# Gancheekim/ATM-VFI

Measured on AMD Instinct MI355X. Metric: interpolated frames/s at 1080p (network_base, bs=1), higher is better.
Workload: dtype f32 (contractions as fp16 hi/lo split x3 MFMA, fp32 accumulate; ~22 significand bits)

## Files before the change

### atm-vfi_amd/csrc/conv3x3_planes.hip

```cpp
#include "conv3_common.h"

#include <stdlib.h>

#ifdef ATMVFI_STAMP
static unsigned long long* g_planes_stamp = nullptr;
extern "C" void atmvfi_debug_set_planes_stamp_buffer(void* p) { g_planes_stamp = (unsigned long long*)p; }
#ifdef ATMVFI_STAMP_KSTEP
#define PDBG(bit) ((a.dbg & (bit)) != 0)
#else
#define PDBG(bit) false
#endif
#define PSTAMP_DECL unsigned long long st_[8] = {0, 0, 0, 0, 0, 0, 0, 0}; unsigned long long st_epi = 0; unsigned long long st_t0 = __builtin_amdgcn_s_memtime();
#define TSTAMP(k) { __builtin_amdgcn_sched_barrier(0); const unsigned long long t1_ = __builtin_amdgcn_s_memtime(); st_[k] += t1_ - st_t0; st_t0 = t1_; __builtin_amdgcn_sched_barrier(0); }
#ifdef ATMVFI_STAMP_KSTEP
#define PSTAMP(k) TSTAMP(k)
#else
#define PSTAMP(k)
#endif
#else
#define PDBG(bit) false
#define PSTAMP_DECL
#define PSTAMP(k)
#define TSTAMP(k)
#endif

namespace {

struct Conv3PDev {
    const _Float16* in_hi;
    const _Float16* in_lo;
    long long in_rows;
    int N, H, W, Cin;
    const _Float16* w_hi;
    const _Float16* w_lo;
    int wrows, cf, tail;
    int Cout;
    float* out;
    int out_ld;
    const float* bias;
    const float* prelu;
    _Float16* out_hi;
    _Float16* out_lo;
    long long plane_rows;
    int out_c0;
    const float* plane_prelu;
    _Float16* out_hi2;
    _Float16* out_lo2;
    long long plane_rows2;
    int out_c02;
    int out_cmin;
    int tiles_x, tiles_y, nblocks, tchunk;
    int vblocks;
    unsigned dm_nblocks, ds_nblocks, dm_perimg, ds_perimg, dm_grp, ds_grp, dm_rows, ds_rows;
    int ksplit, cps;
    long long part_stride;
    const _Float16* h2_w;
    float* h2_out;
    long long h2_plane;
    unsigned long long* stamp;
    int dbg;
};

constexpr int HALO_PIX = HW_ * HW_;
constexpr int HALO_PLANE_PIECES = (HALO_PIX + 15) / 16;
constexpr int HALO_LO = HALO_PLANE_PIECES * 1024;
constexpr int HALO_BYTES = 2 * HALO_LO;

constexpr int planes_const_floats(int BN) { return (3 * BN + 63) / 64 * 64; }
constexpr int ring_slots(int wn) {
    const int free_bytes = 160 * 1024 - 2 * HALO_BYTES - 2 * planes_const_floats(16 * wn) * 4;
    const int n = free_bytes / (2 * 16 * wn * 64);
    return n > 5 ? 5 : n;
}
template <int N>
__device__ __forceinline__ void wait_vm() { asm volatile("s_waitcnt vmcnt(%0)" ::"n"(N) : "memory"); }
__device__ __forceinline__ void dma16(const unsigned char* src, unsigned char* lds_wave_base) {
    __builtin_amdgcn_global_load_lds((const __attribute__((address_space(1))) void*)src,
                                     (__attribute__((address_space(3))) void*)lds_wave_base, 16, 0, 0);
}

template <int BN>
__device__ __forceinline__ void dma_planes_consts(const float* bias, const float* slope, const float* plane_slope, int Cout, int n0, float* cst,
                                                  int wave, int lane) {
    constexpr int NPIECE = (3 * BN + 63) / 64;
    static_assert(NPIECE <= 8, "one piece per wave");
    const int piece = wave % NPIECE;
    const int t = piece * 64 + lane;
    const int row = t / BN;
    const int col = n0 + t - row * BN;
    const float* src = row == 0 ? bias : row == 1 ? slope : plane_slope;
    const float* p = (src && row < 3 && col < Cout) ? src + col : &kEpilogueDefaults[row == 0 ? 0 : 1];
    __builtin_amdgcn_global_load_lds((const __attribute__((address_space(1))) void*)p,
                                     (__attribute__((address_space(3))) void*)(cst + piece * 64), 4, 0, 0);
}

template <int WN>
__global__ __launch_bounds__(512, 1) void conv3x3_planes_kernel(const Conv3PDev a) {
    fp16_saturate_on();
    constexpr int BN = 16 * WN;
    constexpr int WSLOT = 2 * BN * 64;
    constexpr int SW = (2 * WN + 7) / 8;
    constexpr int NB = ring_slots(WN);
    constexpr int LA = NB - 1;
    constexpr int CSTF = planes_const_floats(BN);
    extern __shared__ __attribute__((aligned(16))) unsigned char smem[];
    const unsigned halo0 = lds_offset(smem);
    const unsigned ring0 = halo0 + 2 * HALO_BYTES;
    float* cst_base = reinterpret_cast<float*>(smem + 2 * HALO_BYTES + NB * WSLOT);

    const int tid = threadIdx.x;
    const int lane = tid & 63;
    const int wave = __builtin_amdgcn_readfirstlane(tid >> 6);
    const int grp = wave >> 2;
    const int r = lane & 15;
    const int g = lane >> 4;

    const _Float16* in_hi = a.in_hi;
    const _Float16* in_lo = a.in_lo;
    const _Float16* w_hi = a.w_hi;
    const _Float16* w_lo = a.w_lo;
    float* out_f32 = a.out;
    int nfull = a.cf >> 5;
    int ktail = a.tail;
    if (a.ksplit > 1) {
        const int sp = blockIdx.y;
        const int rem = nfull - a.cps * a.ksplit;
        const int c0 = sp * a.cps + (sp < rem ? sp : rem);
        const bool last = sp == a.ksplit - 1;
        in_hi += (long long)c0 * a.in_rows * 32;
        in_lo += (long long)c0 * a.in_rows * 32;
        w_hi += (long long)c0 * 9 * a.wrows * 32;
        w_lo += (long long)c0 * 9 * a.wrows * 32;
        nfull = a.cps + (sp < rem ? 1 : 0);
        ktail = last ? ktail : 0;
        out_f32 += sp * a.part_stride;
    }

    const int grid = gridDim.x;
    const int per_img = a.tiles_x * a.tiles_y;
    auto fdiv = [](int n, unsigned m, unsigned sh) -> int { return (int)((__umulhi((unsigned)n, m) + (unsigned)n) >> sh); };
    auto decode = [&](int v, int& t_img, int& t_ox0, int& t_oy0, int& t_n0) -> bool {
        int sgrp, nblk, L;
        if (a.ksplit > 1) {
            sgrp = fdiv(v, a.dm_nblocks, a.ds_nblocks);
            nblk = v - sgrp * a.nblocks;
            L = sgrp;
        } else {
            const int slot = v >> 3;
// ... 158 lines not shown
#pragma unroll
            for (int i = 0; i < 2; ++i) {
                const int p = prow + i * HW_ + ((dtail >> (TAIL ? 8 * T : 0)) & 0xff);
                const unsigned addr = halo0 + (unsigned)hcur + (unsigned)(p * 64 + (swz64(p) << 4));
                lds_read16<0>(xh[i], addr);
                lds_read16<HALO_LO>(xl[i], addr);
            }
        }
        const unsigned wa = wfrag + (unsigned)rd_off;
        if (!PDBG(16)) static_for<0, WN>([&](auto jc) {
            constexpr int j = decltype(jc)::value;
            lds_read16<j * 1024>(wh[j], wa);
            lds_read16<j * 1024 + BN * 64>(wl[j], wa);
        });
        rd_off = rd_off + WSLOT == NB * WSLOT ? 0 : rd_off + WSLOT;
        PSTAMP(1)
        if (!PDBG(2)) issue_weights();
        if constexpr (!TAIL && T < 6) {
            if (!PDBG(1)) issue_halo(std::integral_constant<int, T>{});
        }
        if constexpr (TAIL && T < 2) {
            if (!PDBG(1)) {
                issue_halo(std::integral_constant<int, 3 * T>{});
                issue_halo(std::integral_constant<int, 3 * T + 1>{});
                issue_halo(std::integral_constant<int, 3 * T + 2>{});
            }
        }
        PSTAMP(2)
        if constexpr (FIRST && T < LA - 1) {
        } else {
            constexpr int lo = T + 1 - LA > 0 ? T + 1 - LA : 0;
            constexpr int hi = T < 5 ? T : 5;
            constexpr int halos = !TAIL ? (hi >= lo ? hi - lo + 1 : 0) : (lo <= 0 ? 3 : 0) + ((lo <= 1 && T >= 1) ? 3 : 0);
            if (!PDBG(4)) wait_vm<(!TAIL && T == 8) ? (LA - 1) * SW : (LA - 1) * SW + halos>();
        }
        PSTAMP(3)
        asm volatile("s_waitcnt lgkmcnt(0)"
                     : "+v"(xh[0]), "+v"(xh[1]), "+v"(xl[0]), "+v"(xl[1]));
#pragma unroll
        for (int j = 0; j < WN; ++j) asm volatile("" : "+v"(wh[j]), "+v"(wl[j]));
        __builtin_amdgcn_sched_barrier(0);
        PSTAMP(4)
        __builtin_amdgcn_s_barrier();
        __builtin_amdgcn_sched_barrier(0);
        PSTAMP(5)
        if (!PDBG(8)) __builtin_amdgcn_s_setprio(1);
        static_for<0, WN>([&](auto jc) {
            constexpr int j = decltype(jc)::value;
            cor[0][j] = __builtin_amdgcn_mfma_f32_16x16x32_f16(wl[j], xh[0], cor[0][j], 0, 0, 0);
            cor[1][j] = __builtin_amdgcn_mfma_f32_16x16x32_f16(wl[j], xh[1], cor[1][j], 0, 0, 0);
            acc[0][j] = __builtin_amdgcn_mfma_f32_16x16x32_f16(wh[j], xh[0], acc[0][j], 0, 0, 0);
            acc[1][j] = __builtin_amdgcn_mfma_f32_16x16x32_f16(wh[j], xh[1], acc[1][j], 0, 0, 0);
            cor[0][j] = __builtin_amdgcn_mfma_f32_16x16x32_f16(wh[j], xl[0], cor[0][j], 0, 0, 0);
            cor[1][j] = __builtin_amdgcn_mfma_f32_16x16x32_f16(wh[j], xl[1], cor[1][j], 0, 0, 0);
        });
        __builtin_amdgcn_s_setprio(0);
        __builtin_amdgcn_sched_barrier(0);
        PSTAMP(6)
        __builtin_amdgcn_s_barrier();
        __builtin_amdgcn_sched_barrier(0);
        PSTAMP(7)
    };
    auto next_chunk = [&]() {
        const int d = hcur ? -HALO_BYTES : HALO_BYTES;
#pragma unroll
        for (int k = 0; k < 8; ++k) xa[k] += d;
        hcur += d;
        halo_advance();
    };

    constexpr int KK2 = (WN == 2 || WN == 4) ? WN / 2 : 1;
    f16x8 w2h[2][KK2], w2l[2][KK2];
    if constexpr (WN == 2 || WN == 4) {
        if (a.h2_w) {
            const f16x8* wp = reinterpret_cast<const f16x8*>(a.h2_w);
#pragma unroll
            for (int t = 0; t < 2; ++t)
#pragma unroll
                for (int kk = 0; kk < KK2; ++kk) {
                    w2h[t][kk] = wp[(t * KK2 + kk) * 64 + lane];
                    w2l[t][kk] = wp[((2 + t) * KK2 + kk) * 64 + lane];
                }
        }
    }
    for (;;) {
        const float* cst = cst_base + (seq & 1) * CSTF;
#pragma unroll
        for (int i = 0; i < 2; ++i)
#pragma unroll
            for (int j = 0; j < WN; ++j) {
                acc[i][j] = (f32x4){0.f, 0.f, 0.f, 0.f};
                cor[i][j] = (f32x4){0.f, 0.f, 0.f, 0.f};
                asm volatile("" : "+v"(acc[i][j]), "+v"(cor[i][j]));
            }
        if (nfull > 0) {
            static_for<0, 9>([&](auto tc) { kstep(tc, std::false_type{}, std::true_type{}); });
            next_chunk();
        }
        for (int c = 1; c < nfull; ++c) {
            static_for<0, 9>([&](auto tc) { kstep(tc, std::false_type{}, std::false_type{}); });
            next_chunk();
        }
        if (ktail) {
            static_for<0, 3>([&](auto tc) { kstep(tc, std::true_type{}, std::false_type{}); });
            next_chunk();
        }
#if !defined(ATMVFI_STAMP_KSTEP)
        TSTAMP(1)
#endif
        if (grp == 0) __builtin_amdgcn_s_barrier();
        if (has_next) {
            dma_planes_consts<BN>(a.bias, a.prelu, a.plane_prelu, a.Cout, nn0, cst_base + ((seq + 1) & 1) * CSTF, wave, lane);
            wait_vm<1>();
        } else {
            wait_vm<0>();
        }
#if !defined(ATMVFI_STAMP_KSTEP)
        TSTAMP(2)
#endif

    constexpr bool MAXFORM = WN < 8;
    bool slopes_in_range = true;
#pragma unroll
    for (int k = 0; MAXFORM && k < (2 * BN + 63) / 64; ++k) {
        const int idx = BN + 64 * k + lane;
        const float sv = cst[idx < 3 * BN ? idx : 3 * BN - 1];
        slopes_in_range = slopes_in_range && sv >= 0.f && sv <= 1.f;
    }
    const bool pmax = __builtin_amdgcn_ballot_w64(!slopes_in_range) == 0ull;
    auto prelu4 = [](auto mode, const f32x4 v, const f32x4 sl, const bool on) -> f32x4 {
        constexpr int MODE = decltype(mode)::value;
        if constexpr (MODE == 3) {
            f32x4 o = v;
            if (on) o = (f32x4){v.x > 0.f ? v.x : sl.x * v.x, v.y > 0.f ? v.y : sl.y * v.y, v.z > 0.f ? v.z : sl.z * v.z, v.w > 0.f ? v.w : sl.w * v.w};
            return o;
        } else
        if constexpr (MODE == 2) {
            const f32x4 t = sl * v;
            f32x4 o;
            asm("v_max_f32 %0, %1, %2" : "=v"(o.x) : "v"(v.x), "v"(t.x));
            asm("v_max_f32 %0, %1, %2" : "=v"(o.y) : "v"(v.y), "v"(t.y));
            asm("v_max_f32 %0, %1, %2" : "=v"(o.z) : "v"(v.z), "v"(t.z));
            asm("v_max_f32 %0, %1, %2" : "=v"(o.w) : "v"(v.w), "v"(t.w));
            return o;
        } else if constexpr (MODE == 1) {
            return (f32x4){v.x > 0.f ? v.x : sl.x * v.x, v.y > 0.f ? v.y : sl.y * v.y, v.z > 0.f ? v.z : sl.z * v.z, v.w > 0.f ? v.w : sl.w * v.w};
        } else {
            return v;
        }
    };
    typedef std::integral_constant<int, 0> ActNone;
    typedef std::integral_constant<int, 1> ActSelect;
    typedef std::integral_constant<int, 2> ActMax;
    typedef std::integral_constant<int, 3> ActRuntime;
    const int cb = 8 * (g & 1) + 4 * (g >> 1);
    float* orow[2];
    long long prow_o[2];
    bool live[2];
#pragma unroll
    for (int i = 0; i < 2; ++i) {
        const int oy = oy0 + 2 * wave + i, ox = ox0 + r;
        live[i] = oy < a.H && ox < a.W;
        prow_o[i] = ((long long)img * a.H + (live[i] ? oy : 0)) * a.W + (live[i] ? ox : 0);
        orow[i] = out_f32 ? out_f32 + prow_o[i] * a.out_ld : nullptr;
    }
    f32x4 vv[2][WN];
    auto fold = [&](auto mode) {
#pragma unroll
        for (int j = 0; j < WN; ++j) {
            const int cl = 16 * j + cb;
            const f32x4 bv = *reinterpret_cast<const f32x4*>(cst + cl);
            const f32x4 pv = *reinterpret_cast<const f32x4*>(cst + BN + cl);
#pragma unroll
            for (int i = 0; i < 2; ++i) vv[i][j] = prelu4(mode, acc[i][j] + cor[i][j] * LO_UNSCALE + bv, pv, a.prelu != nullptr);
        }
    };
    if constexpr (!MAXFORM) fold(ActRuntime{});
    else if (!a.prelu) fold(ActNone{});
    else if (pmax) fold(ActMax{});
    else fold(ActSelect{});
    if constexpr (WN == 2 || WN == 4) {
        if (a.h2_w) {
            constexpr int KK = WN / 2;
#pragma unroll
            for (int i = 0; i < 2; ++i) {
                f32x4 a2[2] = {(f32x4){0.f, 0.f, 0.f, 0.f}, (f32x4){0.f, 0.f, 0.f, 0.f}};
                f32x4 c2[2] = {(f32x4){0.f, 0.f, 0.f, 0.f}, (f32x4){0.f, 0.f, 0.f, 0.f}};
#pragma unroll
                for (int kk = 0; kk < KK; ++kk) {
                    const f32x4 u0 = vv[i][2 * kk], u1 = vv[i][2 * kk + 1];
                    f16x2 h0, l0, h1, l1, h2, l2, h3, l3;
                    split_pair((f32x2){u0.x, u0.y}, h0, l0);
                    split_pair((f32x2){u0.z, u0.w}, h1, l1);
                    split_pair((f32x2){u1.x, u1.y}, h2, l2);
                    split_pair((f32x2){u1.z, u1.w}, h3, l3);
                    const f16x8 bh = {h0.x, h0.y, h1.x, h1.y, h2.x, h2.y, h3.x, h3.y};
                    const f16x8 bl = {l0.x, l0.y, l1.x, l1.y, l2.x, l2.y, l3.x, l3.y};
#pragma unroll
                    for (int t = 0; t < 2; ++t) {
                        c2[t] = __builtin_amdgcn_mfma_f32_16x16x32_f16(w2l[t][kk], bh, c2[t], 0, 0, 0);
                        a2[t] = __builtin_amdgcn_mfma_f32_16x16x32_f16(w2h[t][kk], bh, a2[t], 0, 0, 0);
                        c2[t] = __builtin_amdgcn_mfma_f32_16x16x32_f16(w2h[t][kk], bl, c2[t], 0, 0, 0);
                    }
                }
#pragma unroll
                for (int t = 0; t < 2; ++t) {
                    const f32x4 tv = a2[t] + c2[t] * LO_UNSCALE;
                    const int row = 16 * t + 4 * g;
                    float* tp = a.h2_out + (long long)row * a.h2_plane + prow_o[i];
                    if (live[i]) {
                        if (row + 0 < 27) tp[0] = tv.x;
                        if (row + 1 < 27) tp[a.h2_plane] = tv.y;
                        if (row + 2 < 27) tp[2 * a.h2_plane] = tv.z;
                        if (row + 3 < 27) tp[3 * a.h2_plane] = tv.w;
                    }
                }
// ... 74 lines not shown
#ifdef ATMVFI_STAMP
        if (a.stamp) {
            __builtin_amdgcn_sched_barrier(0);
            const unsigned long long t_end = __builtin_amdgcn_s_memtime();
            st_epi += t_end - st_t0;
            st_t0 = t_end;
            __builtin_amdgcn_sched_barrier(0);
        }
#endif
        if (!has_next) break;
        vb += grid;
        img = nimg; ox0 = nox0; oy0 = noy0; n0 = nn0;
        ++seq;
        has_next = decode(vb + grid, nimg, nox0, noy0, nn0);
#pragma unroll
        for (int s = 0; s < SW; ++s) wnext[s] = weight_base(s, nn0);
        if (grp == 1) __builtin_amdgcn_s_barrier();
#if !defined(ATMVFI_STAMP_KSTEP)
        TSTAMP(3)
#endif
    }
#ifdef ATMVFI_STAMP
    if (a.stamp && lane == 0) {
        unsigned long long* o = a.stamp + ((long long)blockIdx.x * 8 + wave) * 10;
        const unsigned long long nt = (unsigned long long)(seq + 1);
        o[0] = st_[0];
        for (int k = 1; k < 8; ++k) o[k] = st_[k] / nt;
        o[8] = st_epi / nt;
        o[9] = (unsigned long long)nk;
    }
#endif
}

template <int WN>
int launch_planes(const Conv3PDev& d, int ntiles, hipStream_t s) {
    constexpr int BN = 16 * WN;
    const size_t lds = (size_t)2 * HALO_BYTES + (size_t)ring_slots(WN) * 2 * BN * 64 + 2 * planes_const_floats(BN) * sizeof(float);
    static_assert(2 * HALO_BYTES + ring_slots(WN) * 2 * BN * 64 + 2 * planes_const_floats(BN) * 4 <= 160 * 1024, "LDS budget");
    auto kern = conv3x3_planes_kernel<WN>;
    const hipError_t attr_err = atmvfi::allow_dynamic_lds<conv3x3_planes_kernel<WN>>(lds);
    ATMVFI_REQUIRE(attr_err == hipSuccess, ATMVFI_ELAUNCH, "conv3x3_planes: hipFuncSetAttribute: %s", hipGetErrorString(attr_err));
    Conv3PDev ds = d;
    ds.nblocks = (ntiles + WN - 1) / WN;
    ds.tiles_y = (d.H + 15) / 16;
    const long long sgroups = ((long long)d.N * d.tiles_x * ds.tiles_y + 7) / 8;
    ds.tchunk = (int)sgroups;
#ifdef ATMVFI_STAMP
    ds.stamp = g_planes_stamp;
    static const int dbg = [] { const char* e = getenv("ATMVFI_P3_DBG"); return e ? atoi(e) : 0; }();
    ds.dbg = dbg;
#else
    ds.stamp = nullptr;
    ds.dbg = 0;
#endif
    ATMVFI_REQUIRE(sgroups * 8 * ds.nblocks < (1LL << 31), ATMVFI_EINVAL, "conv3x3_planes: grid too large");
    auto magic = [](int d, unsigned& m, unsigned& sh) {
        sh = 0;
        while ((1ll << sh) < d) ++sh;
        m = (unsigned)((((unsigned long long)1 << (32 + sh)) + (unsigned)d - 1) / (unsigned)d - ((unsigned long long)1 << 32));
    };
    magic(ds.nblocks, ds.dm_nblocks, ds.ds_nblocks);
    magic(d.tiles_x * ds.tiles_y, ds.dm_perimg, ds.ds_perimg);
    magic(8 * d.tiles_x, ds.dm_grp, ds.ds_grp);
    magic((ds.tiles_y & 7) ? (ds.tiles_y & 7) : 8, ds.dm_rows, ds.ds_rows);
    ds.vblocks = d.ksplit > 1 ? (int)((long long)d.N * d.tiles_x * ds.tiles_y * ds.nblocks) : (int)(sgroups * 8 * ds.nblocks);
    const int nchunks = (d.cf >> 5) + (d.tail ? 1 : 0);
    if (d.ksplit > 1) {
        hipLaunchKernelGGL(kern, dim3((unsigned)ds.vblocks, (unsigned)d.ksplit), dim3(512), lds, s, ds);
        return atmvfi::check_launch("conv3x3_planes (split-K)");
    }
    const int grid = nchunks >= 2 ? std::min(ds.vblocks, atmvfi::cu_count()) : ds.vblocks;
    hipLaunchKernelGGL(kern, dim3((unsigned)grid), dim3(512), lds, s, ds);
    return atmvfi::check_launch("conv3x3_planes");
// ... 116 lines not shown
    return conv3x3_planes_impl(in_hi, in_lo, in_rows, N, H, W, Cin, w_hi, w_lo, Cout, out, out_ld, bias, prelu, out_hi, out_lo, plane_rows, out_c0,
                               plane_prelu, out_hi2, out_lo2, plane_rows2, out_c02, out_cmin, wn, workspace, workspace_floats, nullptr, nullptr, 0,
                               stream);
}

static int conv3x3_planes_impl(const void* in_hi, const void* in_lo, int64_t in_rows, int N, int H, int W, int Cin, const void* w_hi,
                               const void* w_lo, int Cout, float* out, int out_ld, const float* bias, const float* prelu, void* out_hi,
                               void* out_lo, int64_t plane_rows, int out_c0, const float* plane_prelu, void* out_hi2, void* out_lo2,
                               int64_t plane_rows2, int out_c02, int out_cmin, int wn, float* workspace, int64_t workspace_floats,
                               const void* h2_w, float* h2_out, int64_t h2_plane, void* stream) {
    ATMVFI_REQUIRE((out_hi2 == nullptr) == (out_lo2 == nullptr), ATMVFI_EINVAL, "conv3x3_planes: the second plane sink needs both planes");
    if (out_hi2)
        ATMVFI_REQUIRE(out_hi && plane_rows2 >= (int64_t)N * H * W && out_c02 >= 0 && out_c02 % 8 == 0 && atmvfi::aligned16(out_hi2) &&
                           atmvfi::aligned16(out_lo2), ATMVFI_EINVAL,
                       "conv3x3_planes: the second plane sink needs the first one, plane_rows2 >= N*H*W, a channel offset that is a multiple "
                       "of 8 and 16-byte aligned planes");
    ATMVFI_REQUIRE(N > 0 && H > 0 && W > 0 && Cin > 0 && Cout > 0, ATMVFI_EINVAL, "conv3x3_planes: bad shape");
    ATMVFI_REQUIRE(in_rows > (int64_t)N * H * W && in_rows * 64 < (1ll << 32), ATMVFI_EINVAL,
                   "conv3x3_planes: in_rows %lld must exceed N*H*W (the zero row) and in_rows * 64 must fit 32 bits", (long long)in_rows);
    ATMVFI_REQUIRE(atmvfi::aligned16(in_hi) && atmvfi::aligned16(in_lo) && atmvfi::aligned16(w_hi) && atmvfi::aligned16(w_lo) &&
                       (!bias || atmvfi::aligned16(bias)) && (!prelu || atmvfi::aligned16(prelu)),
                   ATMVFI_EALIGN, "conv3x3_planes: pointers (incl. bias/prelu) must be 16-byte aligned");
    if (out)
        ATMVFI_REQUIRE(atmvfi::aligned16(out) && out_ld % 4 == 0 && out_cmin >= 0 && out_cmin % 4 == 0 &&
                           out_ld >= atmvfi::round_up(Cout, 4) - out_cmin,
                       ATMVFI_EALIGN, "conv3x3_planes: fp32 output must be 16-byte aligned with ld %% 4 == 0 covering the stored channels");
    ATMVFI_REQUIRE((out_hi == nullptr) == (out_lo == nullptr), ATMVFI_EINVAL, "conv3x3_planes: plane sink needs both planes");
    if (out_hi) {
        ATMVFI_REQUIRE(plane_rows >= (int64_t)N * H * W && out_c0 >= 0 && out_c0 % 8 == 0, ATMVFI_EINVAL,
                       "conv3x3_planes: plane sink needs plane_rows >= N*H*W and a channel offset that is a multiple of 8");
        ATMVFI_REQUIRE(atmvfi::aligned16(out_hi) && atmvfi::aligned16(out_lo) && (!plane_prelu || atmvfi::aligned16(plane_prelu)),
                       ATMVFI_EALIGN, "conv3x3_planes: plane sink pointers must be 16-byte aligned");
    }
    ATMVFI_REQUIRE(wn >= 0 && wn <= 8, ATMVFI_EINVAL, "conv3x3_planes: wn 0 (auto) or 1..8");
    ATMVFI_REQUIRE(out_cmin >= 0 && out_cmin % 4 == 0, ATMVFI_EINVAL, "conv3x3_planes: out_cmin must be a non-negative multiple of 4");
    Conv3PDev d;
    d.in_hi = (const _Float16*)in_hi; d.in_lo = (const _Float16*)in_lo; d.in_rows = in_rows;
    d.N = N; d.H = H; d.W = W; d.Cin = Cin;
    d.w_hi = (const _Float16*)w_hi; d.w_lo = (const _Float16*)w_lo;
    d.wrows = atmvfi::round_up(Cout, 16);
    const int t = Cin % 32;
    if (t >= 1 && t <= 8) { d.cf = Cin - t; d.tail = t; } else { d.cf = atmvfi::round_up(Cin, 32); d.tail = 0; }
    d.Cout = Cout; d.out = out; d.out_ld = out_ld; d.bias = bias; d.prelu = prelu;
    d.out_hi = (_Float16*)out_hi; d.out_lo = (_Float16*)out_lo; d.plane_rows = plane_rows; d.out_c0 = out_c0; d.plane_prelu = plane_prelu;
    d.out_hi2 = (_Float16*)out_hi2; d.out_lo2 = (_Float16*)out_lo2; d.plane_rows2 = plane_rows2; d.out_c02 = out_c02;
    d.out_cmin = out_cmin;
    d.tiles_x = (W + TW - 1) / TW;
    d.tiles_y = 0; d.nblocks = 0; d.tchunk = 0;
    d.h2_w = (const _Float16*)h2_w; d.h2_out = h2_out; d.h2_plane = h2_plane;
    const int ntiles = (Cout + 15) / 16;
    ATMVFI_REQUIRE(!workspace || atmvfi::aligned16(workspace), ATMVFI_EALIGN, "conv3x3_planes: the split-K workspace must be 16-byte aligned");
    Conv3Plan plan = conv3_plan(N, H, W, Cin, Cout, wn, workspace != nullptr);
    const int ldp = atmvfi::round_up(Cout, 16);
    const long long rows = (long long)N * H * W;
    if (plan.ksplit > 1 && (long long)plan.ksplit * rows * ldp > workspace_floats) plan = conv3_plan(N, H, W, Cin, Cout, wn, false);
    d.ksplit = plan.ksplit; d.cps = plan.cps; d.part_stride = rows * ldp;
    const int best = plan.wn;
    Conv3PDev full = d;
    if (plan.ksplit > 1) {
        d.out = workspace; d.out_ld = ldp; d.out_cmin = 0; d.bias = nullptr; d.prelu = nullptr;
        d.out_hi = d.out_lo = d.out_hi2 = d.out_lo2 = nullptr; d.plane_prelu = nullptr;
    }
    hipStream_t s = (hipStream_t)stream;
    int rc;
    switch (best) {
        case 1: rc = launch_planes<1>(d, ntiles, s); break;
        case 2: rc = launch_planes<2>(d, ntiles, s); break;
        case 3: rc = launch_planes<3>(d, ntiles, s); break;
        case 4: rc = launch_planes<4>(d, ntiles, s); break;
        case 5: rc = launch_planes<5>(d, ntiles, s); break;
        case 6: rc = launch_planes<6>(d, ntiles, s); break;
        case 7: rc = launch_planes<7>(d, ntiles, s); break;
        default: rc = launch_planes<8>(d, ntiles, s); break;
    }
    if (rc != ATMVFI_OK || plan.ksplit <= 1) return rc;
    const long long groups = rows * (((Cout + 7) & ~7) >> 2);
    const unsigned blocks = (unsigned)std::min<long long>((groups + 255) / 256, 4096);
    hipLaunchKernelGGL(conv3_splitk_reduce_kernel, dim3(blocks), dim3(256), 0, s, workspace, d.part_stride, plan.ksplit, rows, ldp, Cout,
                       full.bias, full.prelu, full.out, full.out_ld, full.out_cmin, full.out_hi, full.out_lo, (long long)full.plane_rows,
                       full.out_c0, full.plane_prelu, full.out_hi2, full.out_lo2, (long long)full.plane_rows2, full.out_c02);
    return atmvfi::check_launch("conv3x3_planes (split-K reduce)");
}

extern "C" int atmvfi_conv3x3_planes_readout(const void* in_hi, const void* in_lo, int64_t in_rows, int N, int H, int W, int Cin,
                                              const void* w_hi, const void* w_lo, int Cout, const float* bias, const float* prelu,
                                              const void* w2, float* contrib, int64_t contrib_plane, void* stream) {
    ATMVFI_REQUIRE(in_hi && in_lo && w_hi && w_lo && w2 && contrib, ATMVFI_EINVAL, "conv3x3_planes_readout: null pointer");
    ATMVFI_REQUIRE(Cout == 32 || Cout == 64, ATMVFI_EINVAL, "conv3x3_planes_readout: Cout must be 32 or 64 (one column block of 2 or 4 n-tiles), got %d", Cout);
    ATMVFI_REQUIRE(contrib_plane >= (int64_t)N * H * W && atmvfi::aligned16(w2), ATMVFI_EINVAL,
                   "conv3x3_planes_readout: contrib_plane must cover N*H*W pixels and w2 must be 16-byte aligned");
    return conv3x3_planes_impl(in_hi, in_lo, in_rows, N, H, W, Cin, w_hi, w_lo, Cout, nullptr, 0, bias, prelu, nullptr, nullptr, 0, 0, nullptr,
                               nullptr, nullptr, 0, 0, 0, Cout / 16, nullptr, 0, w2, contrib, contrib_plane, stream);
}

extern "C" int atmvfi_conv3x3_planes2(const void* in_hi, const void* in_lo, int64_t in_rows, int N, int H, int W, int Cin, const void* w_hi,
                                       const void* w_lo, int Cout, float* out, int out_ld, const float* bias, const float* prelu,
                                       void* out_hi, void* out_lo, int64_t plane_rows, int out_c0, const float* plane_prelu, void* out_hi2,
                                       void* out_lo2, int64_t plane_rows2, int out_c02, int out_cmin, int wn, void* stream) {
    return atmvfi_conv3x3_planes3(in_hi, in_lo, in_rows, N, H, W, Cin, w_hi, w_lo, Cout, out, out_ld, bias, prelu, out_hi, out_lo, plane_rows,
                                  out_c0, plane_prelu, out_hi2, out_lo2, plane_rows2, out_c02, out_cmin, wn, nullptr, 0, stream);
}

extern "C" int atmvfi_conv3x3_planes(const void* in_hi, const void* in_lo, int64_t in_rows, int N, int H, int W, int Cin, const void* w_hi,
                                      const void* w_lo, int Cout, float* out, int out_ld, const float* bias, const float* prelu,
                                      void* out_hi, void* out_lo, int64_t plane_rows, int out_c0, const float* plane_prelu, int out_cmin,
                                      int wn, void* stream) {
    return atmvfi_conv3x3_planes2(in_hi, in_lo, in_rows, N, H, W, Cin, w_hi, w_lo, Cout, out, out_ld, bias, prelu, out_hi, out_lo, plane_rows,
                                  out_c0, plane_prelu, nullptr, nullptr, 0, 0, out_cmin, wn, stream);
}
```

### atm-vfi_amd/hip_ops.py

```python
from __future__ import annotations

import ctypes
import os
from dataclasses import dataclass
from typing import List, Optional

import torch

_HERE = os.path.dirname(os.path.abspath(__file__))
LIB_PATH = os.path.join(_HERE, "libatmvfi_hip.so")
CHECKED_LIB_PATH = os.path.join(_HERE, "libatmvfi_hip_checked.so")

GEMM_CONV, GEMM_LINEAR, GEMM_DECONV = 0, 1, 2

c_f = ctypes.c_void_p
c_i = ctypes.c_int
C_SLOTS = ctypes.POINTER(ctypes.c_int32)
c_l = ctypes.c_int64


class HipLibraryMissing(RuntimeError):
    pass


# ... 651 lines not shown

        def padded(v, rows, fill):
            out = torch.full((rows,), fill, dtype=torch.float32, device=self.device)
            out[:v.shape[0]] = v.detach().float()
            return out
        r2 = (c0 + 15) // 16 * 16
        w2h, w2l = planes_of(w2, r2)
        w3h, w3l = planes_of(w3, c1)
        k1 = torch.zeros(r2, 32, dtype=torch.float32, device=self.device)
        k1[:c0, :27] = w1.detach().float().permute(0, 2, 3, 1).reshape(c0, 27)
        w1h = k1.half()
        w1l = ((k1 - w1h.float()) * 1024.0).half()
        return StemWeights(c0, c1, w1h, w1l, padded(b1, r2, 0.0), padded(p1, r2, 1.0), w2h, w2l, padded(b2, r2, 0.0), padded(p2, r2, 1.0),
                           w3h, w3l, b3.detach().float().contiguous(), p3.detach().float().contiguous())

    def stem_fused(self, x, w: "StemWeights", out: Planes):
        _chk(x, "stem_fused.x")
        if x.dim() != 4 or x.shape[3] != 4 or not x.is_contiguous():
            raise ValueError(f"stem_fused: expected contiguous NHWC4 frames [F,H,W,4], got {tuple(x.shape)}")
        f, h, wd, _ = x.shape
        if h % 2 or wd % 2 or out.rows != f * (h // 2) * (wd // 2) or out.c != w.c1:
            raise ValueError(f"stem_fused: planes [{out.rows},{out.c}] do not hold {f}x{h // 2}x{wd // 2} pixels x {w.c1} channels")
        if self.precision != "f16x3":
            raise ValueError("stem_fused: needs the f16x3 engine")
        flops = 2.0 * f * h * wd * (27 * w.c0 + 9 * w.c0 * w.c0) + 2.0 * f * (h // 2) * (wd // 2) * 9 * w.c0 * w.c1
        meta = {"flops": flops, "bytes": 16.0 * f * h * wd + 4.0 * out.rows * out.chunks * 32, "shape": f"{f}x{h}x{wd} 3>{w.c0}>{w.c0}>{w.c1}s2"}
        self._run("stem_fused", meta, self.lib.atmvfi_stem_fused, _ptr(x), f, h, wd, w.c0, w.c1, _ptr(w.w1h), _ptr(w.w1l), _ptr(w.b1), _ptr(w.p1),
                  _ptr(w.w2h), _ptr(w.w2l), _ptr(w.b2), _ptr(w.p2), _ptr(w.w3h), _ptr(w.w3l), _ptr(w.b3), _ptr(w.p3),
                  _ptr(out.t[0]), _ptr(out.t[1]), out.ld_rows, self._stream())

    def conv3x3_planes(self, x: Planes, n: int, h: int, wd: int, w: PackedWeight, out=None, bias=None, prelu=None,
                       planes: Optional[Planes] = None, planes_c0: int = 0, planes_prelu=None, in_chunk0: int = 0, cin: Optional[int] = None,
                       wn: int = 0, out_cmin: int = 0, planes2: Optional[Planes] = None, planes2_c0: int = 0,
                       workspace: Optional[torch.Tensor] = None):
        cin = (x.c - 32 * in_chunk0) if cin is None else cin
        if self.precision != "f16x3" or w.hi3 is None:
            raise ValueError("conv3x3_planes: needs the f16x3 engine and the conv3x3 weight planes")
        if w.mode != GEMM_CONV or w.kh != 3 or w.kw != 3 or w.cin != cin:
            raise ValueError(f"conv3x3_planes: weight ({w.cout},{w.cin},{w.kh},{w.kw}) does not match Cin {cin}")
        if x.rows != n * h * wd or x.ld_rows <= x.rows or 32 * in_chunk0 + cin > x.chunks * 32:
            raise ValueError(f"conv3x3_planes: input planes [{x.rows} (+{x.ld_rows - x.rows} spare), {x.c}] do not fit {n}x{h}x{wd} pixels x {cin} channels "
                             "(one spare zero row is required)")
        cout = w.cout
        old = 0
        out_ptr = _ptr(out)
        if out is not None:
            old, on, oh, ow, oc = nhwc_view(out, "conv3x3_planes.out")
            if (on, oh, ow) == (n, h, wd) and oc == cout - out_cmin and out_cmin > 0:
                out_ptr = _ptr(out, -4 * out_cmin)
            elif (on, oh, ow, oc) != (n, h, wd, cout):
                raise ValueError(f"conv3x3_planes: out {tuple(out.shape)} != [{n},{h},{wd},{cout}] (or {cout - out_cmin} channels: compact)")
        elif planes is None:
            raise ValueError("conv3x3_planes: no output")
        if planes is not None:
            if planes.rows != n * h * wd or planes_c0 % 8 or planes_c0 + cout > planes.chunks * 32:
                raise ValueError(f"conv3x3_planes: plane sink [{planes.rows},{planes.c}] cannot take {cout} channels at offset {planes_c0}")
            if planes_prelu is not None and planes_prelu.numel() < (cout + 31) // 32 * 32:
                raise ValueError("conv3x3_planes: planes_prelu must be padded to a multiple of 32 channels")
        if planes2 is not None and (planes is None or planes2.rows != n * h * wd or planes2_c0 % 8 or planes2_c0 + cout > planes2.chunks * 32):
            raise ValueError(f"conv3x3_planes: second plane sink [{planes2.rows},{planes2.c}] needs the first one and room for {cout} channels at {planes2_c0}")
        meta = {"flops": 2.0 * n * h * wd * cout * cin * 9, "bytes": 4.0 * (n * h * wd * (cin + cout) + cout * cin * 9),
                "shape": f"M{n * h * wd} N{cout} K{cin * 9}"}
        coff = in_chunk0 * x.ld_rows * 32 * 2
        if workspace is not None and (workspace.dtype != torch.float32 or not workspace.is_cuda or not workspace.is_contiguous()):
            raise ValueError("conv3x3_planes: the split-K workspace must be a contiguous CUDA fp32 tensor")
        self._run("conv3x3_planes", meta, self.lib.atmvfi_conv3x3_planes3, _ptr(x.t[0], coff), _ptr(x.t[1], coff), x.ld_rows,
                  n, h, wd, cin, _ptr(w.hi3), _ptr(w.lo3), cout, out_ptr, old, _ptr(bias), _ptr(prelu),
                  _ptr(planes.t[0]) if planes is not None else None, _ptr(planes.t[1]) if planes is not None else None,
                  planes.ld_rows if planes is not None else 0, planes_c0, _ptr(planes_prelu) if planes is not None else None,
                  _ptr(planes2.t[0]) if planes2 is not None else None, _ptr(planes2.t[1]) if planes2 is not None else None,
                  planes2.ld_rows if planes2 is not None else 0, planes2_c0, out_cmin, wn, _ptr(workspace),
                  workspace.numel() if workspace is not None else 0, self._stream())

    def pack_readout(self, w: torch.Tensor) -> torch.Tensor:
        o3, c, kh, kw = w.shape
        if (o3, kh, kw) != (3, 3, 3) or c not in (32, 64):
            raise ValueError(f"pack_readout: expected a [3, 32 | 64, 3, 3] weight, got {tuple(w.shape)}")
        w2 = torch.zeros(32, c, dtype=torch.float32, device=self.device)
        w2[:27] = w.detach().float().permute(2, 3, 0, 1).reshape(27, c)
        kk_n = c // 32
        lane = torch.arange(64, device=self.device)
        r, g = lane & 15, lane >> 4
        cb = 8 * (g & 1) + 4 * (g >> 1)
        e = torch.arange(8, device=self.device)
        ch = cb[:, None] + torch.where(e < 4, e, 16 + e - 4)[None, :]
        full = torch.empty(2, kk_n, 64, 8, dtype=torch.float32, device=self.device)
        for t in range(2):
            for kk in range(kk_n):
                full[t, kk] = w2[(16 * t + r)[:, None].expand(64, 8), 32 * kk + ch]
        hi = full.half()
        lo = ((full - hi.float()) * 1024.0).half()
        return torch.stack([hi, lo], 0).contiguous()

    def conv3x3_planes_readout(self, x: Planes, n: int, h: int, wd: int, w: PackedWeight, bias, prelu, w2: torch.Tensor, contrib: torch.Tensor):
        if self.precision != "f16x3" or w.hi3 is None or w.kh != 3 or w.cin > x.chunks * 32 or x.rows != n * h * wd or x.ld_rows <= x.rows:
            raise ValueError("conv3x3_planes_readout: needs the f16x3 engine, conv3x3 weight planes and input planes with a spare zero row")
        if w.cout not in (32, 64) or tuple(w2.shape) != (2, 2, w.cout // 32, 64, 8) or w2.dtype != torch.float16:
            raise ValueError("conv3x3_planes_readout: Cout must be 32 or 64 and w2 the pack_readout() operand of that width")
        if contrib.dtype != torch.float32 or contrib.dim() != 2 or contrib.shape[0] != 27 or contrib.shape[1] < n * h * wd or not contrib.is_contiguous():
            raise ValueError("conv3x3_planes_readout: contrib must be contiguous fp32 [27, >= N*H*W]")
        meta = {"flops": 2.0 * n * h * wd * w.cout * (w.cin * 9 + 27), "bytes": 4.0 * n * h * wd * (w.cin + 27), "shape": f"M{n * h * wd} N{w.cout} K{w.cin * 9} +27"}
        self._run("conv3x3_planes", meta, self.lib.atmvfi_conv3x3_planes_readout, _ptr(x.t[0]), _ptr(x.t[1]), x.ld_rows, n, h, wd, w.cin,
                  _ptr(w.hi3), _ptr(w.lo3), w.cout, _ptr(bias), _ptr(prelu), _ptr(w2), _ptr(contrib), contrib.shape[1], self._stream())

    def refine_tail(self, contrib, bias, slope, it, it_sum, it_clamped):
        _planar(it, 3, "refine_tail.it"); _planar(it_sum, 3, "refine_tail.sum"); _planar(it_clamped, 3, "refine_tail.clamped")
        b, _, h, w = it.shape
        if contrib.dim() != 2 or contrib.shape[0] != 27 or contrib.shape[1] < b * h * w or not contrib.is_contiguous():
            raise ValueError("refine_tail: contrib must be contiguous fp32 [27, >= B*H*W]")
        self._run("refine_tail", {"bytes": 4.0 * b * h * w * (27 + 9)}, self.lib.atmvfi_refine_tail, _ptr(contrib), contrib.shape[1], _ptr(bias),
                  _ptr(slope), _ptr(it), _ptr(it_sum), _ptr(it_clamped), b, h, w, self._stream())

    def conv3x3_workspace_floats(self, n: int, h: int, wd: int, cin: int, cout: int) -> int:
        return int(self.lib.atmvfi_conv3x3_planes_workspace_floats(n, h, wd, cin, cout))

    def head1x1_planes(self, x: Planes, n: int, h: int, wd: int, w: PackedWeight, out, bias=None):
        old, on, oh, ow, oc = nhwc_view(out, "head1x1_planes.out")
        if w.mode != GEMM_CONV or w.kh != 1 or w.cout > 8 or (on, oh, ow, oc) != (n, h, wd, w.cout) or x.rows != n * h * wd or w.cin > x.chunks * 32:
            raise ValueError(f"head1x1_planes: weight ({w.cout},{w.cin},{w.kh},{w.kw}) / out {tuple(out.shape)} / planes [{x.rows},{x.c}] mismatch")
        wt = w.orig.detach()
        if not wt.is_contiguous():
            wt = wt.contiguous()
        meta = {"flops": 2.0 * n * h * wd * w.cout * w.cin, "bytes": 4.0 * n * h * wd * (w.cin + w.cout), "shape": f"M{n * h * wd} N{w.cout} K{w.cin}"}
        self._run("head1x1_planes", meta, self.lib.atmvfi_head1x1_planes, _ptr(x.t[0]), _ptr(x.t[1]), x.ld_rows, n * h * wd, w.cin,
                  _ptr(wt), _ptr(bias), w.cout, _ptr(out), old, self._stream())

    def conv_planes(self, x: Planes, n: int, h: int, wd: int, w: PackedWeight, out=None, stride=1, pad=1, dil=1, bias=None, prelu=None,
                    sink: Optional[Planes] = None, sink_c0: int = 0, in_chunk0: int = 0, x2: Optional[Planes] = None, x2_chunk0: int = 0,
                    split_chunks: int = 0):
        if self.precision != "f16x3" or w.hi is None or w.mode != GEMM_CONV:
            raise ValueError("conv_planes: needs the f16x3 engine and split conv weights")
        cin, cout = w.cin, w.cout
        oh = (h + 2 * pad - dil * (w.kh - 1) - 1) // stride + 1
        ow = (wd + 2 * pad - dil * (w.kw - 1) - 1) // stride + 1
        c1 = 32 * split_chunks if x2 is not None else cin
        for t, c0, cc, what in ((x, in_chunk0, c1, "x"),) + (((x2, x2_chunk0, cin - c1, "x2"),) if x2 is not None else ()):
# ... 591 lines not shown
```

Baseline: 51.83.

## Pair two conv3x3 k-steps per barrier phase for narrow planes kernels

For the WN=1,2,4 conv3x3 planes kernels, the main loop now processes two filter taps per barrier-delimited phase. Each phase issues two weight-slot loads and two halo loads, does one vmcnt wait and runs twice the MFMAs, so the number of workgroup barriers and waits per chunk is halved. The ring grows to six slots with two phases of lookahead. For WN=4 the readout weights are staged in LDS rather than held in registers, to relieve register pressure from the doubled fragment set. A flag bit keeps the old single-k-step path selectable. The change costs more VGPRs for the extra operand fragments and adds odd-chunk handling complexity.

```diff
diff --git a/atm-vfi_amd/csrc/conv3x3_planes.hip b/atm-vfi_amd/csrc/conv3x3_planes.hip
--- a/atm-vfi_amd/csrc/conv3x3_planes.hip
+++ b/atm-vfi_amd/csrc/conv3x3_planes.hip
@@ -5,7 +5,7 @@
 #ifdef ATMVFI_STAMP
 static unsigned long long* g_planes_stamp = nullptr;
 extern "C" void atmvfi_debug_set_planes_stamp_buffer(void* p) { g_planes_stamp = (unsigned long long*)p; }
-#ifdef ATMVFI_STAMP_KSTEP
+#if defined(ATMVFI_STAMP_KSTEP) || defined(ATMVFI_STAMP_DBG)
 #define PDBG(bit) ((a.dbg & (bit)) != 0)
 #else
 #define PDBG(bit) false
@@ -72,6 +72,13 @@
     const int n = free_bytes / (2 * 16 * wn * 64);
     return n > 5 ? 5 : n;
 }
+constexpr int ring_slots_paired(int wn) {
+    const int free_bytes = 160 * 1024 - 2 * HALO_BYTES - 2 * planes_const_floats(16 * wn) * 4;
+    const int n = free_bytes / (2 * 16 * wn * 64);
+    return n > 6 ? 6 : n;
+}
+constexpr bool readout_in_lds(int wn, bool pair) { return pair && wn == 4; }
+constexpr int readout_lds_bytes(int wn, bool pair) { return readout_in_lds(wn, pair) ? 4 * (wn / 2) * 64 * 16 : 0; }
 template <int N>
 __device__ __forceinline__ void wait_vm() { asm volatile("s_waitcnt vmcnt(%0)" ::"n"(N) : "memory"); }
 __device__ __forceinline__ void dma16(const unsigned char* src, unsigned char* lds_wave_base) {
@@ -94,14 +101,16 @@
                                      (__attribute__((address_space(3))) void*)(cst + piece * 64), 4, 0, 0);
 }
 
-template <int WN>
+template <int WN, bool PAIR = false>
 __global__ __launch_bounds__(512, 1) void conv3x3_planes_kernel(const Conv3PDev a) {
     fp16_saturate_on();
+    static_assert(!PAIR || WN <= 4, "paired k-steps: the narrow instances only");
     constexpr int BN = 16 * WN;
     constexpr int WSLOT = 2 * BN * 64;
     constexpr int SW = (2 * WN + 7) / 8;
-    constexpr int NB = ring_slots(WN);
-    constexpr int LA = NB - 1;
+    constexpr int NB = PAIR ? ring_slots_paired(WN) : ring_slots(WN);
+    constexpr int LA = PAIR ? NB - 2 : NB - 1;
+    static_assert(!PAIR || LA == 4, "kstep2's vmcnt counts assume two phases of lookahead");
     constexpr int CSTF = planes_const_floats(BN);
     extern __shared__ __attribute__((aligned(16))) unsigned char smem[];
     const unsigned halo0 = lds_offset(smem);
@@ -114,6 +123,8 @@
     const int grp = wave >> 2;
     const int r = lane & 15;
     const int g = lane >> 4;
+    const int lane_k = lane;
+    auto fresh_lane = [&]() { int l = lane_k; asm volatile("" : "+v"(l)); return l; };
 
     const _Float16* in_hi = a.in_hi;
     const _Float16* in_lo = a.in_lo;
@@ -338,7 +349,8 @@
             constexpr int lo = T + 1 - LA > 0 ? T + 1 - LA : 0;
             constexpr int hi = T < 5 ? T : 5;
             constexpr int halos = !TAIL ? (hi >= lo ? hi - lo + 1 : 0) : (lo <= 0 ? 3 : 0) + ((lo <= 1 && T >= 1) ? 3 : 0);
-            if (!PDBG(4)) wait_vm<(!TAIL && T == 8) ? (LA - 1) * SW : (LA - 1) * SW + halos>();
+            constexpr int WB = PAIR ? LA - 2 : LA - 1;
+            if (!PDBG(4)) wait_vm<((!TAIL && T == 8) || (PAIR && TAIL && T == 2)) ? WB * SW : WB * SW + halos>();
         }
         PSTAMP(3)
         asm volatile("s_waitcnt lgkmcnt(0)"
@@ -367,26 +379,125 @@
         __builtin_amdgcn_sched_barrier(0);
         PSTAMP(7)
     };
-    auto next_chunk = [&]() {
+    auto read_advance = [&]() {
         const int d = hcur ? -HALO_BYTES : HALO_BYTES;
 #pragma unroll
         for (int k = 0; k < 8; ++k) xa[k] += d;
         hcur += d;
+    };
+    auto next_chunk = [&]() {
+        read_advance();
         halo_advance();
     };
 
+    f16x8 xh2[2], xl2[2], wh2[PAIR ? WN : 1], wl2[PAIR ? WN : 1];
+    auto kstep2 = [&](auto tc, auto firstc) {
+        constexpr int T0 = decltype(tc)::value;
+        constexpr int T1 = T0 == 8 ? 0 : T0 + 1;
+        constexpr bool FIRST = decltype(firstc)::value;
+        if (!PDBG(16)) {
+            constexpr int C0 = (T0 / 3) * HW_ + T0 % 3, C1 = C0 + HW_;
+            lds_read16<64 * C0>(xh[0], xa[C0 & 7]);
+            lds_read16<64 * C0 + HALO_LO>(xl[0], xa[C0 & 7]);
+            lds_read16<64 * C1>(xh[1], xa[C1 & 7]);
+            lds_read16<64 * C1 + HALO_LO>(xl[1], xa[C1 & 7]);
+        }
+        if constexpr (T0 == 8) read_advance();
+        if (!PDBG(16)) {
+            constexpr int D0 = (T1 / 3) * HW_ + T1 % 3, D1 = D0 + HW_;
+            lds_read16<64 * D0>(xh2[0], xa[D0 & 7]);
+            lds_read16<64 * D0 + HALO_LO>(xl2[0], xa[D0 & 7]);
+            lds_read16<64 * D1>(xh2[1], xa[D1 & 7]);
+            lds_read16<64 * D1 + HALO_LO>(xl2[1], xa[D1 & 7]);
+        }
+        const unsigned wa = wfrag + (unsigned)rd_off;
+        rd_off = rd_off + WSLOT == NB * WSLOT ? 0 : rd_off + WSLOT;
+        const unsigned wb = wfrag + (unsigned)rd_off;
+        rd_off = rd_off + WSLOT == NB * WSLOT ? 0 : rd_off + WSLOT;
+        if (!PDBG(16)) static_for<0, WN>([&](auto jc) {
+            constexpr int j = decltype(jc)::value;
+            lds_read16<j * 1024>(wh[j], wa);
+            lds_read16<j * 1024 + BN * 64>(wl[j], wa);
+        });
+        if (!PDBG(16)) static_for<0, WN>([&](auto jc) {
+            constexpr int j = decltype(jc)::value;
+            lds_read16<j * 1024>(wh2[j], wb);
+            lds_read16<j * 1024 + BN * 64>(wl2[j], wb);
+        });
+        PSTAMP(1)
+        if (!PDBG(2)) {
+            issue_weights();
+            issue_weights();
+        }
+        if constexpr (T0 < 6) {
+            if (!PDBG(1)) {
+                issue_halo(std::integral_constant<int, (T0 & ~1)>{});
+                issue_halo(std::integral_constant<int, (T0 & ~1) + 1>{});
+            }
+        }
+        PSTAMP(2)
+        if constexpr (!FIRST) {
+            constexpr int halos = (T0 < 6 ? 2 : 0) + ((T0 >= 2 && T0 < 6) ? 2 : 0);
+            if (!PDBG(4)) wait_vm<(LA - 2) * SW + halos>();
+        }
+        PSTAMP(3)
+        asm volatile("s_waitcnt lgkmcnt(0)"
+                     : "+v"(xh[0]), "+v"(xh[1]), "+v"(xl[0]), "+v"(xl[1]), "+v"(xh2[0]), "+v"(xh2[1]), "+v"(xl2[0]), "+v"(xl2[1]));
+#pragma unroll
+        for (int j = 0; j < WN; ++j) asm volatile("" : "+v"(wh[j]), "+v"(wl[j]), "+v"(wh2[j]), "+v"(wl2[j]));
+        __builtin_amdgcn_sched_barrier(0);
+        PSTAMP(4)
+        __builtin_amdgcn_s_barrier();
+        __builtin_amdgcn_sched_barrier(0);
+        PSTAMP(5)
+        if (!PDBG(8)) __builtin_amdgcn_s_setprio(1);
+        static_for<0, WN>([&](auto jc) {
+            constexpr int j = decltype(jc)::value;
+            cor[0][j] = __builtin_amdgcn_mfma_f32_16x16x32_f16(wl[j], xh[0], cor[0][j], 0, 0, 0);
+            cor[1][j] = __builtin_amdgcn_mfma_f32_16x16x32_f16(wl[j], xh[1], cor[1][j], 0, 0, 0);
+            acc[0][j] = __builtin_amdgcn_mfma_f32_16x16x32_f16(wh[j], xh[0], acc[0][j], 0, 0, 0);
+            acc[1][j] = __builtin_amdgcn_mfma_f32_16x16x32_f16(wh[j], xh[1], acc[1][j], 0, 0, 0);
+            cor[0][j] = __builtin_amdgcn_mfma_f32_16x16x32_f16(wh[j], xl[0], cor[0][j], 0, 0, 0);
+            cor[1][j] = __builtin_amdgcn_mfma_f32_16x16x32_f16(wh[j], xl[1], cor[1][j], 0, 0, 0);
+        });
+        static_for<0, WN>([&](auto jc) {
+            constexpr int j = decltype(jc)::value;
+            cor[0][j] = __builtin_amdgcn_mfma_f32_16x16x32_f16(wl2[j], xh2[0], cor[0][j], 0, 0, 0);
+            cor[1][j] = __builtin_amdgcn_mfma_f32_16x16x32_f16(wl2[j], xh2[1], cor[1][j], 0, 0, 0);
+            acc[0][j] = __builtin_amdgcn_mfma_f32_16x16x32_f16(wh2[j], xh2[0], acc[0][j], 0, 0, 0);
+            acc[1][j] = __builtin_amdgcn_mfma_f32_16x16x32_f16(wh2[j], xh2[1], acc[1][j], 0, 0, 0);
+            cor[0][j] = __builtin_amdgcn_mfma_f32_16x16x32_f16(wh2[j], xl2[0], cor[0][j], 0, 0, 0);
+            cor[1][j] = __builtin_amdgcn_mfma_f32_16x16x32_f16(wh2[j], xl2[1], cor[1][j], 0, 0, 0);
+        });
+        __builtin_amdgcn_s_setprio(0);
+        __builtin_amdgcn_sched_barrier(0);
+        PSTAMP(6)
+        __builtin_amdgcn_s_barrier();
+        __builtin_amdgcn_sched_barrier(0);
+        PSTAMP(7)
+    };
+
     constexpr int KK2 = (WN == 2 || WN == 4) ? WN / 2 : 1;
+    constexpr bool W2LDS = readout_in_lds(WN, PAIR);
     f16x8 w2h[2][KK2], w2l[2][KK2];
+    f16x8* w2s = reinterpret_cast<f16x8*>(smem + 2 * HALO_BYTES + NB * WSLOT + 2 * CSTF * 4);
     if constexpr (WN == 2 || WN == 4) {
         if (a.h2_w) {
             const f16x8* wp = reinterpret_cast<const f16x8*>(a.h2_w);
-#pragma unroll
-            for (int t = 0; t < 2; ++t)
-#pragma unroll
-                for (int kk = 0; kk < KK2; ++kk) {
-                    w2h[t][kk] = wp[(t * KK2 + kk) * 64 + lane];
-                    w2l[t][kk] = wp[((2 + t) * KK2 + kk) * 64 + lane];
+            if constexpr (W2LDS) {
+                if (wave == 0) {
+#pragma unroll
+                    for (int q = 0; q < 4 * KK2; ++q) w2s[q * 64 + lane] = wp[q * 64 + lane];
                 }
+            } else {
+#pragma unroll
+                for (int t = 0; t < 2; ++t)
+#pragma unroll
+                    for (int kk = 0; kk < KK2; ++kk) {
+                        w2h[t][kk] = wp[(t * KK2 + kk) * 64 + lane];
+                        w2l[t][kk] = wp[((2 + t) * KK2 + kk) * 64 + lane];
+                    }
+            }
         }
     }
     for (;;) {
@@ -399,6 +510,34 @@
                 cor[i][j] = (f32x4){0.f, 0.f, 0.f, 0.f};
                 asm volatile("" : "+v"(acc[i][j]), "+v"(cor[i][j]));
             }
+        if constexpr (PAIR) {
+            typedef std::integral_constant<int, 8> Tap8;
+            bool first = true;
+            for (int c = 0; c + 2 <= nfull; c += 2) {
+                if (first) kstep2(std::integral_constant<int, 0>{}, std::true_type{});
+                else kstep2(std::integral_constant<int, 0>{}, std::false_type{});
+                first = false;
+                kstep2(std::integral_constant<int, 2>{}, std::false_type{});
+                kstep2(std::integral_constant<int, 4>{}, std::false_type{});
+                kstep2(std::integral_constant<int, 6>{}, std::false_type{});
+                kstep2(Tap8{}, std::false_type{});
+                halo_advance();
+                kstep2(std::integral_constant<int, 1>{}, std::false_type{});
+                kstep2(std::integral_constant<int, 3>{}, std::false_type{});
+                kstep2(std::integral_constant<int, 5>{}, std::false_type{});
+                kstep2(std::integral_constant<int, 7>{}, std::false_type{});
+                next_chunk();
+            }
+            if (nfull & 1) {
+                if (first) kstep2(std::integral_constant<int, 0>{}, std::true_type{});
+                else kstep2(std::integral_constant<int, 0>{}, std::false_type{});
+                kstep2(std::integral_constant<int, 2>{}, std::false_type{});
+                kstep2(std::integral_constant<int, 4>{}, std::false_type{});
+                kstep2(std::integral_constant<int, 6>{}, std::false_type{});
+                kstep(Tap8{}, std::false_type{}, std::false_type{});
+                next_chunk();
+            }
+        } else {
         if (nfull > 0) {
             static_for<0, 9>([&](auto tc) { kstep(tc, std::false_type{}, std::true_type{}); });
             next_chunk();
@@ -406,6 +545,7 @@
         for (int c = 1; c < nfull; ++c) {
             static_for<0, 9>([&](auto tc) { kstep(tc, std::false_type{}, std::false_type{}); });
             next_chunk();
+        }
         }
         if (ktail) {
             static_for<0, 3>([&](auto tc) { kstep(tc, std::true_type{}, std::false_type{}); });
@@ -425,6 +565,8 @@
         TSTAMP(2)
 #endif
 
+    const int lane = PAIR ? fresh_lane() : lane_k;
+    const int r = lane & 15, g = lane >> 4;
     constexpr bool MAXFORM = WN < 8;
     bool slopes_in_range = true;
 #pragma unroll
@@ -488,6 +630,15 @@
     if constexpr (WN == 2 || WN == 4) {
         if (a.h2_w) {
             constexpr int KK = WN / 2;
+            if constexpr (W2LDS) {
+#pragma unroll
+                for (int t = 0; t < 2; ++t)
+#pragma unroll
+                    for (int kk = 0; kk < KK2; ++kk) {
+                        w2h[t][kk] = w2s[(t * KK2 + kk) * 64 + lane];
+                        w2l[t][kk] = w2s[((2 + t) * KK2 + kk) * 64 + lane];
+                    }
+            }
 #pragma unroll
             for (int i = 0; i < 2; ++i) {
                 f32x4 a2[2] = {(f32x4){0.f, 0.f, 0.f, 0.f}, (f32x4){0.f, 0.f, 0.f, 0.f}};
@@ -628,13 +779,14 @@
 #endif
 }
 
-template <int WN>
+template <int WN, bool PAIR = false>
 int launch_planes(const Conv3PDev& d, int ntiles, hipStream_t s) {
     constexpr int BN = 16 * WN;
-    const size_t lds = (size_t)2 * HALO_BYTES + (size_t)ring_slots(WN) * 2 * BN * 64 + 2 * planes_const_floats(BN) * sizeof(float);
-    static_assert(2 * HALO_BYTES + ring_slots(WN) * 2 * BN * 64 + 2 * planes_const_floats(BN) * 4 <= 160 * 1024, "LDS budget");
-    auto kern = conv3x3_planes_kernel<WN>;
-    const hipError_t attr_err = atmvfi::allow_dynamic_lds<conv3x3_planes_kernel<WN>>(lds);
+    constexpr int NB = PAIR ? ring_slots_paired(WN) : ring_slots(WN);
+    const size_t lds = (size_t)2 * HALO_BYTES + (size_t)NB * 2 * BN * 64 + 2 * planes_const_floats(BN) * sizeof(float) + readout_lds_bytes(WN, PAIR);
+    static_assert(2 * HALO_BYTES + NB * 2 * BN * 64 + 2 * planes_const_floats(BN) * 4 + readout_lds_bytes(WN, PAIR) <= 160 * 1024, "LDS budget");
+    auto kern = conv3x3_planes_kernel<WN, PAIR>;
+    const hipError_t attr_err = atmvfi::allow_dynamic_lds<conv3x3_planes_kernel<WN, PAIR>>(lds);
     ATMVFI_REQUIRE(attr_err == hipSuccess, ATMVFI_ELAUNCH, "conv3x3_planes: hipFuncSetAttribute: %s", hipGetErrorString(attr_err));
     Conv3PDev ds = d;
     ds.nblocks = (ntiles + WN - 1) / WN;
@@ -817,7 +969,9 @@
         ATMVFI_REQUIRE(atmvfi::aligned16(out_hi) && atmvfi::aligned16(out_lo) && (!plane_prelu || atmvfi::aligned16(plane_prelu)),
                        ATMVFI_EALIGN, "conv3x3_planes: plane sink pointers must be 16-byte aligned");
     }
-    ATMVFI_REQUIRE(wn >= 0 && wn <= 8, ATMVFI_EINVAL, "conv3x3_planes: wn 0 (auto) or 1..8");
+    const bool single_kstep = wn >= 0 && (wn & 16) != 0;
+    if (single_kstep) wn &= 15;
+    ATMVFI_REQUIRE(wn >= 0 && wn <= 8, ATMVFI_EINVAL, "conv3x3_planes: wn 0 (auto) or 1..8, | 16 for the single-k-step body");
     ATMVFI_REQUIRE(out_cmin >= 0 && out_cmin % 4 == 0, ATMVFI_EINVAL, "conv3x3_planes: out_cmin must be a non-negative multiple of 4");
     Conv3PDev d;
     d.in_hi = (const _Float16*)in_hi; d.in_lo = (const _Float16*)in_lo; d.in_rows = in_rows;
@@ -849,10 +1003,10 @@
     hipStream_t s = (hipStream_t)stream;
     int rc;
     switch (best) {
-        case 1: rc = launch_planes<1>(d, ntiles, s); break;
-        case 2: rc = launch_planes<2>(d, ntiles, s); break;
+        case 1: rc = single_kstep ? launch_planes<1>(d, ntiles, s) : launch_planes<1, true>(d, ntiles, s); break;
+        case 2: rc = single_kstep ? launch_planes<2>(d, ntiles, s) : launch_planes<2, true>(d, ntiles, s); break;
         case 3: rc = launch_planes<3>(d, ntiles, s); break;
-        case 4: rc = launch_planes<4>(d, ntiles, s); break;
+        case 4: rc = single_kstep ? launch_planes<4>(d, ntiles, s) : launch_planes<4, true>(d, ntiles, s); break;
         case 5: rc = launch_planes<5>(d, ntiles, s); break;
         case 6: rc = launch_planes<6>(d, ntiles, s); break;
         case 7: rc = launch_planes<7>(d, ntiles, s); break;
@@ -871,11 +1025,13 @@
                                               const void* w_hi, const void* w_lo, int Cout, const float* bias, const float* prelu,
                                               const void* w2, float* contrib, int64_t contrib_plane, void* stream) {
     ATMVFI_REQUIRE(in_hi && in_lo && w_hi && w_lo && w2 && contrib, ATMVFI_EINVAL, "conv3x3_planes_readout: null pointer");
+    const int single_kstep = (Cout > 0 && (Cout & 65536)) ? 16 : 0;
+    if (single_kstep) Cout &= 65535;
     ATMVFI_REQUIRE(Cout == 32 || Cout == 64, ATMVFI_EINVAL, "conv3x3_planes_readout: Cout must be 32 or 64 (one column block of 2 or 4 n-tiles), got %d", Cout);
     ATMVFI_REQUIRE(contrib_plane >= (int64_t)N * H * W && atmvfi::aligned16(w2), ATMVFI_EINVAL,
                    "conv3x3_planes_readout: contrib_plane must cover N*H*W pixels and w2 must be 16-byte aligned");
     return conv3x3_planes_impl(in_hi, in_lo, in_rows, N, H, W, Cin, w_hi, w_lo, Cout, nullptr, 0, bias, prelu, nullptr, nullptr, 0, 0, nullptr,
-                               nullptr, nullptr, 0, 0, 0, Cout / 16, nullptr, 0, w2, contrib, contrib_plane, stream);
+                               nullptr, nullptr, 0, 0, 0, Cout / 16 | single_kstep, nullptr, 0, w2, contrib, contrib_plane, stream);
 }
 
 extern "C" int atmvfi_conv3x3_planes2(const void* in_hi, const void* in_lo, int64_t in_rows, int N, int H, int W, int Cin, const void* w_hi,
diff --git a/atm-vfi_amd/hip_ops.py b/atm-vfi_amd/hip_ops.py
--- a/atm-vfi_amd/hip_ops.py
+++ b/atm-vfi_amd/hip_ops.py
@@ -707,7 +707,7 @@
     def conv3x3_planes(self, x: Planes, n: int, h: int, wd: int, w: PackedWeight, out=None, bias=None, prelu=None,
                        planes: Optional[Planes] = None, planes_c0: int = 0, planes_prelu=None, in_chunk0: int = 0, cin: Optional[int] = None,
                        wn: int = 0, out_cmin: int = 0, planes2: Optional[Planes] = None, planes2_c0: int = 0,
-                       workspace: Optional[torch.Tensor] = None):
+                       workspace: Optional[torch.Tensor] = None, single_kstep: bool = False):
         cin = (x.c - 32 * in_chunk0) if cin is None else cin
         if self.precision != "f16x3" or w.hi3 is None:
             raise ValueError("conv3x3_planes: needs the f16x3 engine and the conv3x3 weight planes")
@@ -744,7 +744,7 @@
                   _ptr(planes.t[0]) if planes is not None else None, _ptr(planes.t[1]) if planes is not None else None,
                   planes.ld_rows if planes is not None else 0, planes_c0, _ptr(planes_prelu) if planes is not None else None,
                   _ptr(planes2.t[0]) if planes2 is not None else None, _ptr(planes2.t[1]) if planes2 is not None else None,
-                  planes2.ld_rows if planes2 is not None else 0, planes2_c0, out_cmin, wn, _ptr(workspace),
+                  planes2.ld_rows if planes2 is not None else 0, planes2_c0, out_cmin, wn | (16 if single_kstep else 0), _ptr(workspace),
                   workspace.numel() if workspace is not None else 0, self._stream())
 
     def pack_readout(self, w: torch.Tensor) -> torch.Tensor:
@@ -767,7 +767,8 @@
         lo = ((full - hi.float()) * 1024.0).half()
         return torch.stack([hi, lo], 0).contiguous()
 
-    def conv3x3_planes_readout(self, x: Planes, n: int, h: int, wd: int, w: PackedWeight, bias, prelu, w2: torch.Tensor, contrib: torch.Tensor):
+    def conv3x3_planes_readout(self, x: Planes, n: int, h: int, wd: int, w: PackedWeight, bias, prelu, w2: torch.Tensor, contrib: torch.Tensor,
+                               single_kstep: bool = False):
         if self.precision != "f16x3" or w.hi3 is None or w.kh != 3 or w.cin > x.chunks * 32 or x.rows != n * h * wd or x.ld_rows <= x.rows:
             raise ValueError("conv3x3_planes_readout: needs the f16x3 engine, conv3x3 weight planes and input planes with a spare zero row")
         if w.cout not in (32, 64) or tuple(w2.shape) != (2, 2, w.cout // 32, 64, 8) or w2.dtype != torch.float16:
@@ -776,7 +777,8 @@
             raise ValueError("conv3x3_planes_readout: contrib must be contiguous fp32 [27, >= N*H*W]")
         meta = {"flops": 2.0 * n * h * wd * w.cout * (w.cin * 9 + 27), "bytes": 4.0 * n * h * wd * (w.cin + 27), "shape": f"M{n * h * wd} N{w.cout} K{w.cin * 9} +27"}
         self._run("conv3x3_planes", meta, self.lib.atmvfi_conv3x3_planes_readout, _ptr(x.t[0]), _ptr(x.t[1]), x.ld_rows, n, h, wd, w.cin,
-                  _ptr(w.hi3), _ptr(w.lo3), w.cout, _ptr(bias), _ptr(prelu), _ptr(w2), _ptr(contrib), contrib.shape[1], self._stream())
+                  _ptr(w.hi3), _ptr(w.lo3), w.cout | (65536 if single_kstep else 0), _ptr(bias), _ptr(prelu), _ptr(w2), _ptr(contrib), contrib.shape[1],
+                  self._stream())
 
     def refine_tail(self, contrib, bias, slope, it, it_sum, it_clamped):
         _planar(it, 3, "refine_tail.it"); _planar(it_sum, 3, "refine_tail.sum"); _planar(it_clamped, 3, "refine_tail.clamped")
```

After: 51.94 (median of 6 runs). Within noise of the previous version (+0.2%).
